# Murmeldyret/cubesat-APDS

Measured on AMD Instinct MI355X. Metric: frames/sec (detect+match+homography) 4k×4k tile vs 1M-desc DB; Mmatches/sec, higher is better.
Workload: dtype fp4 e2m1 operands / f32 accumulate = exact integer Hamming (match), f32 (AKAZE), f64 (homography solve)

## Files before the change

### cubesat-apds_amd/csrc/hamming_mfma.hip

```cpp
#include <atomic>
#include <memory>

#include "config.h"
#include "kernels.h"
#include "topk_keys.h"

namespace apds {

typedef int hm_v8i __attribute__((ext_vector_type(8)));
typedef float hm_f32x4 __attribute__((ext_vector_type(4)));
typedef uint32_t hm_u32x4 __attribute__((ext_vector_type(4)));

#ifndef APDS_HM_WAVES
#define APDS_HM_WAVES 8
#endif
static constexpr int HM_WAVES = APDS_HM_WAVES;
static constexpr int HM_TM = 16 * HM_WAVES;
#ifndef APDS_HM_WPE
#define APDS_HM_WPE 4
#endif
#ifndef APDS_HM_NC
#define APDS_HM_NC 3
#endif
static constexpr int HM_NC = APDS_HM_NC;
static constexpr int HM_Q = HM_WAVES * 16 * HM_NC;
static constexpr int HM_UNIT_SCALE = 0x7F7F7F7F;
static constexpr int HM_BIAS = 1024;

__device__ __forceinline__ uint32_t hm_spread8(uint32_t b, uint32_t nib) {
    uint32_t t = b & 0xFFu;
    t = (t | (t << 12)) & 0x000F000Fu;
    t = (t | (t << 6)) & 0x03030303u;
    t = (t | (t << 3)) & 0x11111111u;
    return t * nib;
}

__global__ __launch_bounds__(256) void hm_expand_rows_kernel(const uint32_t* __restrict__ rows, long long n, uint32_t nib, int bias, uint4* __restrict__ out,
                                                             float* __restrict__ pc) {
    APDS_RAISE_WAVE_PRIORITY();
    const long long i = (long long)blockIdx.x * 256 + threadIdx.x;
    const uint32_t d = i < n * 16 ? rows[i] : 0u;
    int v = __popc(d);
#pragma unroll
    for (int off = 8; off > 0; off >>= 1) v += __shfl_xor(v, off);
    if (i >= n * 16) return;
    out[i] = make_uint4(hm_spread8(d, nib), hm_spread8(d >> 8, nib), hm_spread8(d >> 16, nib), hm_spread8(d >> 24, nib));
    if ((threadIdx.x & 15) == 0) pc[i >> 4] = (float)(v + bias);
}

__global__ void hm_pad_rows_kernel(uint4* __restrict__ rows, float* __restrict__ pc, long long n, long long n_pad) {
    const long long i = n + (threadIdx.x >> 4);
    if (i >= n_pad) return;
    for (long long r = i; r < n_pad; r += 8) {
        rows[r * 16 + (threadIdx.x & 15)] = make_uint4(0, 0, 0, 0);
        if ((threadIdx.x & 15) == 0) pc[r] = INFINITY;
    }
}

__global__ void hm_thresholds_kernel(const uint64_t* __restrict__ topk, int K, const float* __restrict__ qpc, int nq, uint32_t* __restrict__ thr) {
    const int i = blockIdx.x * blockDim.x + threadIdx.x;
    if (i >= nq) return;
    const uint64_t k2 = topk[(size_t)i * K + K - 1];
    thr[i] = k2 == EMPTY_KEY ? 0x7F800000u : __float_as_uint((float)((int)key_rank(k2) - (int)qpc[i] + HM_BIAS));
}

struct HmTop2 {
    uint32_t d0, d1;
    uint32_t i0, i1;
};
__device__ __forceinline__ void hm_insert(HmTop2& b, uint32_t d, uint32_t idx) {
    if (d < b.d1) {
        if (d < b.d0) {
            b.d1 = b.d0;
            b.i1 = b.i0;
            b.d0 = d;
            b.i0 = idx;
        } else {
            b.d1 = d;
            b.i1 = idx;
        }
    }
}

__device__ __forceinline__ void hm_dma_rows(const unsigned char* tile_base, const int (&voff)[4], uint32_t lds_dst) {
    uint32_t keep;
    asm volatile(
        "s_mov_b32 %0, m0\n\t"
        "s_mov_b32 m0, %6\n\t"
        "s_nop 0\n\t"
        "global_load_lds_dwordx4 %1, %5\n\t"
        "global_load_lds_dwordx4 %2, %5 offset:1024\n\t"
        "global_load_lds_dwordx4 %3, %5 offset:2048\n\t"
        "global_load_lds_dwordx4 %4, %5 offset:3072\n\t"
        "s_mov_b32 m0, %0"
        : "=&s"(keep)
        : "v"(voff[0]), "v"(voff[1]), "v"(voff[2]), "v"(voff[3]), "s"(tile_base), "s"(lds_dst)
        : "memory");
}
__device__ __forceinline__ void hm_dma_popcounts(const float* src, int voff, uint32_t lds_dst) {
    uint32_t keep;
    asm volatile(
        "s_mov_b32 %0, m0\n\t"
        "s_mov_b32 m0, %3\n\t"
        "s_nop 0\n\t"
        "global_load_lds_dword %1, %2\n\t"
        "s_mov_b32 m0, %0"
        : "=&s"(keep)
        : "v"(voff), "s"(src), "s"(lds_dst)
        : "memory");
}
__device__ __forceinline__ void hm_dma_wait() { asm volatile("s_waitcnt vmcnt(0)" ::: "memory"); }
template <class T>
__device__ __forceinline__ void hm_settle(T& v) { asm volatile("" : "+v"(v)); }

template <int NC, int PRIO, class Rank>
__device__ __forceinline__ void hm_scan_tiles(const uint4* __restrict__ train_fp4, const float* __restrict__ tpc, int tile_begin, int tile_end,
// ... 45 lines not shown
            if (PRIO) __builtin_amdgcn_s_setprio(PRIO);
#pragma unroll
            for (int s = 0; s < 4; s++) {
                const hm_v8i A = {(int)a[s].x, (int)a[s].y, (int)a[s].z, (int)a[s].w, 0, 0, 0, 0};
#pragma unroll
                for (int c = 0; c < NC; c++) {
                    const hm_v8i Bv = {(int)B[c][s].x, (int)B[c][s].y, (int)B[c][s].z, (int)B[c][s].w, 0, 0, 0, 0};
                    acc[c] = __builtin_amdgcn_mfma_scale_f32_16x16x128_f8f6f4(A, Bv, s == 0 ? init : acc[c], 4, 4, 0, HM_UNIT_SCALE, 0, HM_UNIT_SCALE);
                }
            }
            if (PRIO) __builtin_amdgcn_s_setprio(0);
            if (rb + 1 < HM_TM / 16) {
                read_block(rb + 1);
            } else {
                hm_dma_wait();
                __syncthreads();
#pragma unroll
                for (int s = 0; s < 4; s++) ra[s] += buf ? -TILE_BYTES : TILE_BYTES;
                rn += buf ? -HM_TM * 4 : HM_TM * 4;
                read_block(0);
            }
#pragma unroll
            for (int c = 0; c < NC; c++) hm_settle(acc[c]);
            __builtin_amdgcn_sched_barrier(0);
            rank(acc, (uint32_t)(tile * HM_TM + rb * 16 + 4 * kq) + index_base);
        }
    }
}

struct HmItem {
    int split, q0, tile_begin, tile_end;
    int col, kq;
};
template <int NC>
__device__ __forceinline__ HmItem hm_work_item(int n_train, int tiles_per_split, int q_tiles, int splits) {
    const int tid = threadIdx.x, lane = tid & 63, wave = tid >> 6;
    HmItem w;
    int qtile;
    if ((splits & 7) == 0) {
        const int xcd = blockIdx.x & 7, j = blockIdx.x >> 3;
        w.split = xcd + 8 * (j / q_tiles);
        qtile = j % q_tiles;
    } else {
        w.split = blockIdx.x / q_tiles;
        qtile = blockIdx.x % q_tiles;
    }
    w.q0 = qtile * (HM_WAVES * 16 * NC) + wave * 16 * NC;
    const int n_tiles = (n_train + HM_TM - 1) / HM_TM;
    w.tile_begin = w.split * tiles_per_split, w.tile_end = min(n_tiles, w.tile_begin + tiles_per_split);
    w.col = lane & 15, w.kq = lane >> 4;
    return w;
}
template <int NC>
__device__ __forceinline__ void hm_load_queries(const uint4* query_fp4, const float* qpc, int nq, int q0, int col, int kq, uint4 (&B)[NC][4], float (&qq)[NC]) {
#pragma unroll
    for (int c = 0; c < NC; c++) {
        const int qi = min(q0 + 16 * c + col, nq - 1);
#pragma unroll
        for (int s = 0; s < 4; s++) B[c][s] = query_fp4[(size_t)qi * 16 + 4 * s + kq];
        qq[c] = qpc[qi];
    }
}
template <bool THR>
__device__ __forceinline__ uint32_t hm_start_value(const uint32_t* thr, int qi) {
    return THR ? thr[qi] : 0x7F800000u;
}
__device__ __forceinline__ uint32_t hm_distance(float qq, uint32_t d) { return (uint32_t)((int)(qq + __uint_as_float(d)) - HM_BIAS); }

template <int PRIO, bool THR>
__global__ __launch_bounds__(64 * HM_WAVES) __attribute__((amdgpu_waves_per_eu(APDS_HM_WPE, APDS_HM_WPE))) void hamming_mfma_kernel(const uint4* __restrict__ train_fp4, const float* __restrict__ tpc, int n_train,
                                                           const uint4* __restrict__ query_fp4, const float* __restrict__ qpc, int nq, int tiles_per_split,
                                                           int q_tiles, int splits, uint32_t index_base, const uint32_t* __restrict__ thr,
                                                           uint64_t* __restrict__ out) {
    const HmItem w = hm_work_item<HM_NC>(n_train, tiles_per_split, q_tiles, splits);
    const int split = w.split, q0 = w.q0, tile_begin = w.tile_begin, tile_end = w.tile_end, col = w.col, kq = w.kq;
    uint4 B[HM_NC][4];
    float qq[HM_NC];
    hm_load_queries<HM_NC>(query_fp4, qpc, nq, q0, col, kq, B, qq);
    HmTop2 best[HM_NC];
#pragma unroll
    for (int c = 0; c < HM_NC; c++) {
        best[c].d0 = hm_start_value<THR>(thr, min(q0 + 16 * c + col, nq - 1));
        hm_settle(best[c].d0), hm_settle(qq[c]);
        best[c].d1 = best[c].d0;
        best[c].i0 = best[c].i1 = 0xFFFFFFFFu;
    }

    if (tile_begin < tile_end) {
        hm_scan_tiles<HM_NC, PRIO>(train_fp4, tpc, tile_begin, tile_end, B, index_base, [&](const hm_f32x4 (&a)[HM_NC], uint32_t row0) {
            bool hit[HM_NC];
#pragma unroll
            for (int c = 0; c < HM_NC; c++) {
                const uint32_t mn = min(min(__float_as_uint(a[c][0]), __float_as_uint(a[c][1])), min(__float_as_uint(a[c][2]), __float_as_uint(a[c][3])));
                hit[c] = mn < best[c].d1;
            }
#pragma unroll
            for (int c = 0; c < HM_NC; c++)
                if (__any(hit[c])) {
#pragma unroll
                    for (int j = 0; j < 4; j++) hm_insert(best[c], __float_as_uint(a[c][j]), row0 + j);
                }
        });
    }
#pragma unroll
    for (int c = 0; c < HM_NC; c++) {
        HmTop2 b = best[c];
#pragma unroll
        for (int off = 16; off < 64; off <<= 1) {
            const uint32_t od0 = (uint32_t)__shfl_xor((int)b.d0, off), od1 = (uint32_t)__shfl_xor((int)b.d1, off);
            const uint32_t oi0 = (uint32_t)__shfl_xor((int)b.i0, off), oi1 = (uint32_t)__shfl_xor((int)b.i1, off);
            HmTop2 m = b;
            auto ins = [&](uint32_t d, uint32_t i) {
                if (i == 0xFFFFFFFFu) return;
                if (d < m.d0 || (d == m.d0 && i < m.i0)) {
                    m.d1 = m.d0;
                    m.i1 = m.i0;
                    m.d0 = d;
                    m.i0 = i;
                } else if ((d < m.d1 || (d == m.d1 && i < m.i1)) && i != m.i0) {
                    m.d1 = d;
                    m.i1 = i;
                }
            };
            ins(od0, oi0);
            ins(od1, oi1);
            b = m;
        }
        const int qi = q0 + 16 * c + col;
        if (kq == 0 && qi < nq) {
            uint64_t* o = out + ((size_t)split * nq + qi) * 2;
            o[0] = b.i0 == 0xFFFFFFFFu ? EMPTY_KEY : make_key(hm_distance(qq[c], b.d0), b.i0);
            o[1] = b.i1 == 0xFFFFFFFFu ? EMPTY_KEY : make_key(hm_distance(qq[c], b.d1), b.i1);
        }
    }
}

template <int K>
struct HmTopK {
    uint32_t d[K];
    uint32_t i[K];
};
template <int K>
__device__ __forceinline__ void hm_insert_k(HmTopK<K>& b, uint32_t d, uint32_t idx) {
#pragma unroll
    for (int j = K - 1; j > 0; j--) {
        const bool shift = d < b.d[j - 1], here = d < b.d[j];
        b.i[j] = shift ? b.i[j - 1] : (here ? idx : b.i[j]);
        b.d[j] = shift ? b.d[j - 1] : (here ? d : b.d[j]);
    }
    const bool first = d < b.d[0];
    b.i[0] = first ? idx : b.i[0];
    b.d[0] = first ? d : b.d[0];
}
__device__ __forceinline__ uint64_t hm_shfl_xor_u64(uint64_t v, int off) {
    return ((uint64_t)(uint32_t)__shfl_xor((int)(uint32_t)(v >> 32), off) << 32) | (uint32_t)__shfl_xor((int)(uint32_t)v, off);
}

#ifndef APDS_HM_NC_K4
#define APDS_HM_NC_K4 2
#endif
#ifndef APDS_HM_NC_K8
#define APDS_HM_NC_K8 2
#endif
template <int K>
struct HmShape {
    static constexpr int NC = K <= 4 ? APDS_HM_NC_K4 : APDS_HM_NC_K8;
    static constexpr int Q = HM_WAVES * 16 * NC;
};

template <int K, int NC, int PRIO, bool THR>
__global__ __launch_bounds__(64 * HM_WAVES) __attribute__((amdgpu_waves_per_eu(APDS_HM_WPE, APDS_HM_WPE))) void hamming_mfma_topk_kernel(
    const uint4* __restrict__ train_fp4, const float* __restrict__ tpc, int n_train, const uint4* __restrict__ query_fp4, const float* __restrict__ qpc, int nq,
    int tiles_per_split, int q_tiles, int splits, uint32_t index_base, const uint32_t* __restrict__ thr, uint64_t* __restrict__ out) {
    const HmItem w = hm_work_item<NC>(n_train, tiles_per_split, q_tiles, splits);
    const int split = w.split, q0 = w.q0, tile_begin = w.tile_begin, tile_end = w.tile_end, col = w.col, kq = w.kq;
    uint4 B[NC][4];
    float qq[NC];
    hm_load_queries<NC>(query_fp4, qpc, nq, q0, col, kq, B, qq);
    HmTopK<K> best[NC];
#pragma unroll
    for (int c = 0; c < NC; c++) {
        uint32_t start = hm_start_value<THR>(thr, min(q0 + 16 * c + col, nq - 1));
        hm_settle(start), hm_settle(qq[c]);
#pragma unroll
        for (int j = 0; j < K; j++) best[c].d[j] = start, best[c].i[j] = 0xFFFFFFFFu;
    }

    if (tile_begin < tile_end) {
        hm_scan_tiles<NC, PRIO>(train_fp4, tpc, tile_begin, tile_end, B, index_base, [&](const hm_f32x4 (&a)[NC], uint32_t row0) {
            bool hit[NC];
#pragma unroll
            for (int c = 0; c < NC; c++) {
                const uint32_t mn = min(min(__float_as_uint(a[c][0]), __float_as_uint(a[c][1])), min(__float_as_uint(a[c][2]), __float_as_uint(a[c][3])));
                hit[c] = mn < best[c].d[K - 1];
            }
#pragma unroll
            for (int c = 0; c < NC; c++)
                if (__any(hit[c])) {
#pragma unroll
                    for (int j = 0; j < 4; j++) {
                        const uint32_t v = __float_as_uint(a[c][j]);
                        if (__any(v < best[c].d[K - 1])) hm_insert_k<K>(best[c], v, row0 + j);
                    }
                }
        });
    }
#pragma unroll
    for (int c = 0; c < NC; c++) {
        uint64_t key[K];
#pragma unroll
        for (int j = 0; j < K; j++) key[j] = ((uint64_t)best[c].d[j] << 32) | best[c].i[j];
#pragma unroll
        for (int off = 16; off < 64; off <<= 1) {
            uint64_t other[K];
#pragma unroll
            for (int j = 0; j < K; j++) other[j] = hm_shfl_xor_u64(key[j], off);
#pragma unroll
            for (int j = 0; j < K; j++) key[j] = min(key[j], other[K - 1 - j]);
#pragma unroll
            for (int step = K / 2; step > 0; step >>= 1)
#pragma unroll
                for (int j = 0; j < K; j++)
                    if ((j & step) == 0) {
                        const uint64_t lo = min(key[j], key[j + step]), hi = max(key[j], key[j + step]);
                        key[j] = lo;
                        key[j + step] = hi;
                    }
        }
        const int qi = q0 + 16 * c + col;
        if (kq == 0 && qi < nq) {
            uint64_t* o = out + ((size_t)split * nq + qi) * K;
#pragma unroll
            for (int j = 0; j < K; j++) {
                const uint32_t d = key_rank(key[j]), i = key_index(key[j]);
                o[j] = i == 0xFFFFFFFFu ? EMPTY_KEY : make_key(hm_distance(qq[c], d), i);
            }
        }
    }
}

static int hm_list_len(int k) { return k <= 2 ? 2 : (k <= 4 ? 4 : 8); }
static int hm_queries_per_block(int K) { return K <= 2 ? HM_Q : (K <= 4 ? HmShape<4>::Q : HmShape<8>::Q); }

HmPlan hm_plan(int nq, long long nt, int K) {
    HmPlan p;
    p.q_tiles = ceil_div(nq, hm_queries_per_block(K));
    const int t_tiles = (int)ceil_div(nt, (long long)HM_TM);
    constexpr int SLOTS = 256 * (16 / HM_WAVES);
    constexpr int OVERHEAD = 4;
    const int max_splits = (int)std::max<long long>(1, std::min<long long>(std::min(t_tiles, 128), (32ll << 20) / std::max(K, 2) / std::max(nq, 1)));
    long long best_cost = -1;
    p.splits = 1;
    for (int sp = 1; sp <= max_splits; sp++) {
        const long long rounds = ceil_div((long long)p.q_tiles * sp, (long long)SLOTS);
        const long long cost = rounds * (ceil_div(t_tiles, sp) + OVERHEAD);
        if (best_cost < 0 || cost < best_cost) best_cost = cost, p.splits = sp;
    }
    if (config().match_mfma_xcd && t_tiles >= 64) {
        long long best8 = -1;
        int sp8 = 0;
        for (int sp = 8; sp <= std::min(max_splits, 32); sp += 8) {
            const long long rounds = ceil_div((long long)p.q_tiles * sp, (long long)SLOTS);
            const long long cost = rounds * (ceil_div(t_tiles, sp) + OVERHEAD);
            if (best8 < 0 || cost < best8) best8 = cost, sp8 = sp;
        }
        if (sp8 && best8 * 100 <= best_cost * 105) {
            p.splits = sp8;
            p.tiles_per_split = ceil_div(t_tiles, p.splits);
            return p;
        }
    }
    if (config().match_mfma_splits > 0) p.splits = std::min(t_tiles, config().match_mfma_splits);
    p.tiles_per_split = ceil_div(t_tiles, p.splits);
    p.splits = ceil_div(t_tiles, p.tiles_per_split);
    return p;
}

void hm_expand_device(const void* rows64, long long n, bool query, void* out_fp4, float* pc, hipStream_t s) {
    if (n <= 0) return;
    hipLaunchKernelGGL(hm_expand_rows_kernel, dim3((unsigned)ceil_div(n * 16, 256)), dim3(256), 0, s, static_cast<const uint32_t*>(rows64), n, query ? 0xCu : 0x2u,
                       query ? 0 : HM_BIAS, static_cast<uint4*>(out_fp4), pc);
    if (!query && hm_padded_rows(n) > n)
        hipLaunchKernelGGL(hm_pad_rows_kernel, dim3(1), dim3(128), 0, s, static_cast<uint4*>(out_fp4), pc, n, hm_padded_rows(n));
}
long long hm_padded_rows(long long n) { return ceil_div(n, (long long)HM_TM) * HM_TM; }
long long hm_sample_rows(long long nt) {
    const long long cap = config().match_mfma_sample;
    return (cap > 0 && nt >= 65536) ? std::min<long long>(cap, nt / 16 / HM_TM * HM_TM) / HM_TM * HM_TM : 0;
}

template <class... Kernel>
static void hm_opt_in_lds(std::atomic<bool> (&opted_dev)[64], Kernel... kernel) {
    std::atomic<bool>& opted = opted_dev[ctx().device & 63];
    if (opted.load()) return;
    (HIP_CHECK(hipFuncSetAttribute(reinterpret_cast<const void*>(kernel), hipFuncAttributeMaxDynamicSharedMemorySize, 160 * 1024)), ...);
    opted.store(true);
}

template <int K, class Go>
static void hm_scan_k_launch(Go&& go, bool thr) {
    constexpr int NC = HmShape<K>::NC;
    static std::atomic<bool> opted_dev[64];
    hm_opt_in_lds(opted_dev, &hamming_mfma_topk_kernel<K, NC, 0, false>, &hamming_mfma_topk_kernel<K, NC, 2, false>,
                  &hamming_mfma_topk_kernel<K, NC, 0, true>, &hamming_mfma_topk_kernel<K, NC, 2, true>);
    const bool prio = config().match_mfma_prio > 0;
    if (thr) prio ? go(&hamming_mfma_topk_kernel<K, NC, 2, true>) : go(&hamming_mfma_topk_kernel<K, NC, 0, true>);
    else prio ? go(&hamming_mfma_topk_kernel<K, NC, 2, false>) : go(&hamming_mfma_topk_kernel<K, NC, 0, false>);
}

void hm_scan_device(const void* q_fp4, const float* qpc, int nq, const void* t_fp4, const float* tpc, long long nt, const HmPlan& p, uint32_t index_base,
                    uint64_t* parts, hipStream_t s, const uint32_t* thr, bool timed, int K) {
    APDS_REQUIRE(K <= 2 || K == 4 || K == 8, APDS_ERR_ASSERT, "the matrix-core matcher keeps lists of 2, 4 or 8");
    const size_t lds = (size_t)2 * HM_TM * 256 + 2 * HM_TM * sizeof(float) + (size_t)std::max(0, config().match_mfma_lds_pad);
    auto go = [&](auto kernel) {
        hipLaunchKernelGGL(kernel, dim3((unsigned)p.q_tiles * p.splits), dim3(64 * HM_WAVES), lds, s, static_cast<const uint4*>(t_fp4), tpc, (int)nt,
                           static_cast<const uint4*>(q_fp4), qpc, nq, p.tiles_per_split, p.q_tiles, p.splits, index_base, thr, parts);
    };
    std::unique_ptr<KernelTimer> timer, timer_k;
    if (timed) timer.reset(new KernelTimer("hamming_topk", s));
    if (timed && K > 2) timer_k.reset(new KernelTimer("hamming_topk_mfma_k", s));
    if (K == 4) return hm_scan_k_launch<4>(go, thr != nullptr);
    if (K == 8) return hm_scan_k_launch<8>(go, thr != nullptr);
    static std::atomic<bool> opted_dev[64];
    hm_opt_in_lds(opted_dev, &hamming_mfma_kernel<0, false>, &hamming_mfma_kernel<1, false>, &hamming_mfma_kernel<2, false>, &hamming_mfma_kernel<3, false>,
                  &hamming_mfma_kernel<0, true>, &hamming_mfma_kernel<1, true>, &hamming_mfma_kernel<2, true>, &hamming_mfma_kernel<3, true>);
    const int prio = std::max(0, std::min(3, config().match_mfma_prio));
    if (thr) {
        switch (prio) {
            case 0: go(&hamming_mfma_kernel<0, true>); break;
            case 1: go(&hamming_mfma_kernel<1, true>); break;
            case 2: go(&hamming_mfma_kernel<2, true>); break;
            default: go(&hamming_mfma_kernel<3, true>); break;
        }
    } else {
        switch (prio) {
            case 0: go(&hamming_mfma_kernel<0, false>); break;
            case 1: go(&hamming_mfma_kernel<1, false>); break;
            case 2: go(&hamming_mfma_kernel<2, false>); break;
            default: go(&hamming_mfma_kernel<3, false>); break;
        }
    }
}

void* hm_train_create(const void* rows64, long long n, hipStream_t s) {
    APDS_REQUIRE(rows64 && n > 0 && n < (1ll << 31), APDS_ERR_ASSERT, "an expanded train set needs rows");
    HmTrain* t = new HmTrain();
    t->device = ctx().device;
    t->src = rows64;
    t->n = n;
    if (hipMalloc(&t->rows, (size_t)hm_padded_rows(n) * 256) != hipSuccess || hipMalloc(reinterpret_cast<void**>(&t->pc), (size_t)hm_padded_rows(n) * 4) != hipSuccess) {
        (void)hipGetLastError();
        if (t->rows) (void)hipFree(t->rows);
        delete t;
        fail(APDS_ERR_NOMEM, "no device memory for the expanded train rows");
    }
    hm_expand_device(rows64, n, false, t->rows, t->pc, s);
    HIP_CHECK(hipStreamSynchronize(s));
    return t;
}
void hm_train_destroy(void* h) {
    HmTrain* t = static_cast<HmTrain*>(h);
    if (!t) return;
    int previous = -1;
    if (hipGetDevice(&previous) != hipSuccess) previous = -1;
    (void)hipSetDevice(t->device);
    (void)hipDeviceSynchronize();
    if (t->rows) (void)hipFree(t->rows);
    if (t->pc) (void)hipFree(t->pc);
    delete t;
    if (previous >= 0) (void)hipSetDevice(previous);
}

static void hm_topk_expanded(const void* q, int nq, const void* t4, const float* tp, long long nt, uint32_t index_base, int k, uint64_t* out, hipStream_t s) {
    ThreadCtx& c = ctx();
    void* q4 = c.alloc((size_t)nq * 256);
    float* qp = c.alloc_n<float>(nq);
    {
        KernelTimer timer("hamming_topk_sample", s);
        hm_expand_device(q, nq, true, q4, qp, s);
    }
    const long long sample = hm_sample_rows(nt);
    const int K = hm_list_len(k);
    uint64_t* topk = k == K ? out : c.alloc_n<uint64_t>((size_t)nq * K);
    const HmPlan p = hm_plan(nq, nt - sample, K);
    const int lists = p.splits + (sample ? 1 : 0);
    uint64_t* parts = lists == 1 ? topk : c.alloc_n<uint64_t>((size_t)lists * nq * K);
    uint32_t* thr = nullptr;
    if (sample) {
        const HmPlan pa = hm_plan(nq, sample, K);
        uint64_t* parts_a = c.alloc_n<uint64_t>((size_t)pa.splits * nq * K);
        uint64_t* topk_a = parts + (size_t)p.splits * nq * K;
        thr = c.alloc_n<uint32_t>(nq);
        KernelTimer timer("hamming_topk_sample", s);
        hm_scan_device(q4, qp, nq, t4, tp, sample, pa, index_base, parts_a, s, nullptr, false, K);
        if (pa.splits > 1) merge_topk_device(parts_a, pa.splits, nq, K, topk_a, s);
        else HIP_CHECK(hipMemcpyAsync(topk_a, parts_a, (size_t)nq * K * 8, hipMemcpyDeviceToDevice, s));
        hipLaunchKernelGGL(hm_thresholds_kernel, dim3(ceil_div(nq, 256)), dim3(256), 0, s, (const uint64_t*)topk_a, K, (const float*)qp, nq, thr);
    }
    hm_scan_device(q4, qp, nq, static_cast<const char*>(t4) + (size_t)sample * 256, tp + sample, nt - sample, p, index_base + (uint32_t)sample, parts, s, thr,
                   true, K);
    if (lists > 1) merge_topk_device(parts, lists, nq, K, topk, s);
    if (k != K) take_first_columns_device(topk, nq, K, k, out, s);
    HIP_CHECK(hipGetLastError());
}

void hamming_mfma_topk_device(const void* q, int nq, const void* t, long long nt, uint32_t index_base, int k, uint64_t* out, hipStream_t s) {
    APDS_REQUIRE(k >= 1 && k <= 8, APDS_ERR_ASSERT, "the matrix-core matcher serves 1 <= k <= 8");
    APDS_REQUIRE(nq > 0 && nt > 0 && nt < (1ll << 31), APDS_ERR_ASSERT, "the matrix-core matcher needs queries and train rows");
    ThreadCtx& c = ctx();
    void* t4 = c.alloc((size_t)hm_padded_rows(nt) * 256);
    float* tp = c.alloc_n<float>(hm_padded_rows(nt));
    {
        KernelTimer timer("hamming_topk_sample", s);
        hm_expand_device(t, nt, false, t4, tp, s);
    }
    hm_topk_expanded(q, nq, t4, tp, nt, index_base, k, out, s);
}

void hamming_mfma_topk_train_device(const void* q, int nq, const void* train, uint32_t index_base, int k, uint64_t* out, hipStream_t s) {
    const HmTrain* t = static_cast<const HmTrain*>(train);
    APDS_REQUIRE(t && k >= 1 && k <= 8 && nq > 0, APDS_ERR_ASSERT, "the matrix-core matcher needs an expanded train set, queries and 1 <= k <= 8");
    hm_topk_expanded(q, nq, t->rows, t->pc, t->n, index_base, k, out, s);
}

}
```

### cubesat-apds_amd/csrc/kernels.h

```cpp
#pragma once
#include <atomic>
#include "common.h"

namespace apds {

void hamming_topk_device(const void* q, int nq, const void* t, long long nt, uint32_t index_base, int k, uint64_t* out, hipStream_t s, int backend = 0);
void* topk_split_create();
void topk_split_destroy(void* state);
void topk_split_prepass(void* state, const void* q, int nq, const void* t, long long nt, uint32_t index_base, int k, hipStream_t s);
void topk_split_scan(void* state, const void* q, const void* t, hipStream_t s);
void topk_split_merge(void* state, uint32_t index_base, uint64_t* out, hipStream_t s);
void topk_split_use_train(void* state, const void* hm_train);
void pack_rows_device(const void* src, long long n, int desc_bytes, long long src_stride, void* dst, hipStream_t s);
std::atomic<int>& match_lds_cap();
std::atomic<int>& last_scan_launch_lds();
void set_thread_scan_cap(int bytes);

void merge_topk_device(const uint64_t* parts, int nparts, int nq, int k, uint64_t* out, hipStream_t s);
void take_first_columns_device(const uint64_t* in, int nq, int kin, int kout, uint64_t* out, hipStream_t s);

void hamming_mfma_topk_device(const void* q, int nq, const void* t, long long nt, uint32_t index_base, int k, uint64_t* out, hipStream_t s);
struct HmPlan {
    int q_tiles, splits, tiles_per_split;
};
struct HmTrain {
    int device = 0;
    const void* src = nullptr;
    long long n = 0;
    void* rows = nullptr;
    float* pc = nullptr;
};
HmPlan hm_plan(int nq, long long nt, int K = 2);
long long hm_padded_rows(long long n);
void hm_expand_device(const void* rows64, long long n, bool query, void* out_fp4, float* pc, hipStream_t s);
void hm_scan_device(const void* q_fp4, const float* qpc, int nq, const void* t_fp4, const float* tpc, long long nt, const HmPlan& p, uint32_t index_base,
                    uint64_t* parts, hipStream_t s, const uint32_t* thr = nullptr, bool timed = true, int K = 2);
long long hm_sample_rows(long long nt);
void* hm_train_create(const void* rows64, long long n, hipStream_t s);
void hm_train_destroy(void* train);
void hamming_mfma_topk_train_device(const void* q, int nq, const void* train, uint32_t index_base, int k, uint64_t* out, hipStream_t s);

int* scan_flags_device(const uint8_t* flags, int n, int** total_dev, hipStream_t s);
int ratio_filter_device(const uint64_t* keys, int nq, int k, float fs, apds_dmatch* out, hipStream_t s);
int cross_check_device(const uint64_t* train_best, long long n_train, int nq, apds_dmatch* out, hipStream_t s);

double valu_popcount_peak_device();
int valu_peak_modes();
const char* valu_peak_mode_name(int mode);
void valu_peak_device(int mode, int waves_per_simd, double* lane_ops_per_s, double* cycles_per_inst);

int akaze_extract_device(const void* img, int rows, int cols, int channels, size_t stride, int max_points, apds_keypoint* kps,
                         uint8_t* desc64, int capacity, hipStream_t s);
int akaze_extract_batch_device(const void* img, int n_img, size_t img_bstride, int rows, int cols, int channels, size_t stride, int max_points,
                               apds_keypoint* kps, uint8_t* desc64, int capacity, int* counts, hipStream_t s);

void points_from_matches_device(const apds_keypoint* kp1, int n1, const apds_keypoint* kp2, int n2, const apds_dmatch* m, int nm,
                                int bug_compatible, float* pts1, float* pts2, int* err_flag, hipStream_t s);
void rgba_to_bgra_device(const uint8_t* rgba, size_t n_pixels, uint8_t* bgra, hipStream_t s);
int count_nonzero_device(const uint8_t* bytes, int n, int* count_dev, hipStream_t s);

void band_merger_device(const float* r, const float* g, const float* b, size_t n, const double* mm, int bgra, uint8_t* out, hipStream_t s);
void warp_perspective_device(const uint8_t* src, int rows, int cols, const double* M, int dst_rows, int dst_cols, uint8_t* dst, hipStream_t s);
void warp_perspective_any_device(const void* src, int rows, int cols, int channels, int elem_bytes, const double* M, int dst_rows, int dst_cols, void* dst,
                                 hipStream_t s);
int world_coordinates_device(const double* xy, int n, const double* dgt_host, const double* egt_host, const double* elev, int ew, int eh, double* xyz,
                             hipStream_t s);

struct Mosaic;
void mosaic_check_window(const Mosaic* m, int level, const int32_t* xy0, int n_tiles, int win_w, int win_h, int out_w, int out_h, int resample);
void mosaic_read_device(const Mosaic* m, const int32_t* xy0, int n_tiles, int win_w, int win_h, int out_w, int out_h, int resample, float* out, hipStream_t s);
void mosaic_min_max(Mosaic* m, double* minmax6);

int find_homography_device(const float* src, const float* dst, int n, int method, double thr, int max_iters, double confidence,
                           double* H_host, uint8_t* mask_dev, hipStream_t s);

void l2_row_norms_device(const float* x, long long n, int dim, float* out, hipStream_t s);
void l2_topk_device(const float* q, int nq, const float* t, long long nt, int dim, uint32_t index_base, int k, uint64_t* out, hipStream_t s);
bool l2_topk_screen_device(const float* q, int nq, const float* t, long long nt, int dim, uint32_t index_base, int k, uint64_t* out, hipStream_t s,
                           double* candidates_per_query);

int find_homography_rho_device(const float* src, const float* dst, int n, double thr, int max_iters, double confidence, double* H_host, uint8_t* mask_dev,
                               hipStream_t s);

int pnp_ransac_device(const double* obj_xyz, const double* img_xy, int n, const double* K, int iterations, float reproj_thr, double confidence, int method,
                      double* rvec, double* tvec, int32_t* inliers, int* n_inliers, hipStream_t s);
int pnp_ransac_core(const float* obj_dev, const float* img_dev, int n, const double* K, int iterations, float reproj_thr, double confidence, int method,
                    double* rvec, double* tvec, int32_t* inliers, int* n_inliers, hipStream_t s);
int pnp_checked_method(int n, int method);
// ... 9 lines not shown
```

### cubesat-apds_amd/csrc/match_hamming.hip

```cpp
#include <atomic>

#include "config.h"
#include "kernels.h"
#include "popcount_row.h"
#include "topk_keys.h"

namespace apds {

typedef uint32_t u32x4 __attribute__((ext_vector_type(4)));

static constexpr int INF_THR = 1 << 20;
static constexpr uint32_t NO_INDEX = 0xFFFFFFFFu;
static constexpr int PART_ROW_BITS = 22;
template <int T, int K>
struct PartRecord {
    static constexpr int SLOTS = T * K;
    static constexpr int HEADER = 2 * SLOTS;
    static constexpr int PITCH = HEADER + 64 * SLOTS;
};

#ifndef APDS_PAIR_NOP
#define APDS_PAIR_NOP 1
#endif
template <int T>
// ... 433 lines not shown
                   reinterpret_cast<uint32_t*>(buf + L.off_parts), L.p, s, "hamming_topk", floor_keys, floor_base);
}

template <int K>
static void scan_merge(const ScanLayout& L, const char* buf, uint32_t index_base, uint64_t* out, hipStream_t s) {
    merge_records_launch<K>(reinterpret_cast<const uint32_t*>(buf + L.off_parts), L.p, index_base + (uint32_t)L.sample,
                            L.sample ? reinterpret_cast<const uint64_t*>(buf + L.off_sample_keys) : nullptr, L.nq, out, s);
    HIP_CHECK(hipGetLastError());
}

template <int K>
static void topk_device_k(const void* q, int nq, const void* t, long long nt, uint32_t index_base, uint64_t* out, hipStream_t s) {
    const ScanLayout L = scan_layout<K>(nq, nt, false);
    char* buf = static_cast<char*>(ctx().alloc(L.bytes));
    scan_prepass<K>(L, buf, q, t, index_base, s);
    scan_main<K>(L, buf, q, t, s);
    scan_merge<K>(L, buf, index_base, out, s);
}

__global__ void gather_pages_kernel(const uint64_t* __restrict__ pages, int nq, int n_pages, int k, uint64_t* __restrict__ out) {
    const long long i = (long long)blockIdx.x * blockDim.x + threadIdx.x;
    if (i >= (long long)nq * k) return;
    const int q = (int)(i / k), c = (int)(i - (long long)q * k);
    const int page = c >> 4;
    out[i] = page < n_pages ? pages[((size_t)page * nq + q) * 16 + (c & 15)] : EMPTY_KEY;
}

static void topk_paged_device(const void* q, int nq, const void* t, long long nt, uint32_t index_base, int k, uint64_t* out, hipStream_t s) {
    constexpr int K = 16;
    ThreadCtx& c = ctx();
    const int n_pages = (int)std::min<long long>(ceil_div(k, K), ceil_div(nt, K));
    const ScanLayout L = scan_layout<K>(nq, nt, true);
    char* buf = static_cast<char*>(c.alloc(L.bytes));
    uint64_t* pages = c.alloc_n<uint64_t>((size_t)n_pages * nq * K);
    for (int j = 0; j < n_pages; j++) {
        const uint64_t* floor_keys = j ? pages + (size_t)(j - 1) * nq * K : nullptr;
        scan_prepass<K>(L, buf, q, t, index_base, s, floor_keys, index_base);
        scan_main<K>(L, buf, q, t, s, floor_keys, index_base + (uint32_t)L.sample);
        scan_merge<K>(L, buf, index_base, pages + (size_t)j * nq * K, s);
    }
    hipLaunchKernelGGL(gather_pages_kernel, dim3((unsigned)ceil_div((long long)nq * k, 256)), dim3(256), 0, s, (const uint64_t*)pages, nq, n_pages, k, out);
    HIP_CHECK(hipGetLastError());
}

struct TopkSplitState {
    int device = 0;
    char* buf = nullptr;
    size_t cap = 0;
    ScanLayout L{};
    bool mfma = false;
    HmPlan hp{};
    const HmTrain* shared_train = nullptr;
    uint32_t index_base_mfma = 0;
    size_t off_q4 = 0, off_qp = 0, off_t4 = 0, off_tp = 0, off_lists = 0, off_top2 = 0;
    const void* t4 = nullptr;
    const float* tp = nullptr;
};

static void split_reserve(TopkSplitState& st, size_t need) {
    if (need <= st.cap) return;
    HIP_CHECK(hipDeviceSynchronize());
    if (st.buf) (void)hipFree(st.buf);
    st.buf = nullptr;
    st.cap = 0;
    const size_t want = need + need / 4;
    HIP_CHECK(hipMalloc(reinterpret_cast<void**>(&st.buf), want));
    st.cap = want;
}

static void split_prepass_mfma(TopkSplitState& st, const void* q, int nq, const void* t, long long nt, int k, hipStream_t s) {
    st.mfma = true;
    st.L = ScanLayout{};
    st.L.nq = nq, st.L.k = k, st.L.nt = nt;
    st.hp = hm_plan(nq, nt);
    const bool shared = st.shared_train && st.shared_train->src == t && st.shared_train->n == nt;
    size_t need = 0;
    auto take = [&](size_t bytes) {
        const size_t o = need;
        need += (bytes + 255) & ~(size_t)255;
        return o;
    };
    st.off_q4 = take((size_t)nq * 256);
    st.off_qp = take((size_t)nq * 4);
    st.off_lists = take((size_t)st.hp.splits * nq * 16);
    st.off_top2 = take((size_t)nq * 16);
    if (!shared) {
        st.off_t4 = take((size_t)hm_padded_rows(nt) * 256);
        st.off_tp = take((size_t)hm_padded_rows(nt) * 4);
    }
    split_reserve(st, need);
    KernelTimer timer("hamming_topk_sample", s);
    hm_expand_device(q, nq, true, st.buf + st.off_q4, reinterpret_cast<float*>(st.buf + st.off_qp), s);
    if (shared) {
        st.t4 = st.shared_train->rows;
        st.tp = st.shared_train->pc;
    } else {
        hm_expand_device(t, nt, false, st.buf + st.off_t4, reinterpret_cast<float*>(st.buf + st.off_tp), s);
        st.t4 = st.buf + st.off_t4;
        st.tp = reinterpret_cast<const float*>(st.buf + st.off_tp);
    }
    HIP_CHECK(hipGetLastError());
}
static void split_scan_mfma(TopkSplitState& st, hipStream_t s) {
    hm_scan_device(st.buf + st.off_q4, reinterpret_cast<const float*>(st.buf + st.off_qp), st.L.nq, st.t4, st.tp, st.L.nt, st.hp, st.index_base_mfma,
                   reinterpret_cast<uint64_t*>(st.buf + st.off_lists), s);
}
static void split_merge_mfma(TopkSplitState& st, uint64_t* out, hipStream_t s) {
    const int nq = st.L.nq, k = st.L.k;
    const uint64_t* parts = reinterpret_cast<const uint64_t*>(st.buf + st.off_lists);
    uint64_t* top2 = k == 2 ? out : reinterpret_cast<uint64_t*>(st.buf + st.off_top2);
    if (st.hp.splits > 1) merge_topk_device(parts, st.hp.splits, nq, 2, top2, s);
    else if (k == 2) HIP_CHECK(hipMemcpyAsync(out, parts, (size_t)nq * 16, hipMemcpyDeviceToDevice, s));
    else top2 = const_cast<uint64_t*>(parts);
    if (k == 1) take_first_columns_device(top2, nq, 2, 1, out, s);
    HIP_CHECK(hipGetLastError());
}

template <int K>
static void split_prepass_k(TopkSplitState& st, const void* q, int nq, const void* t, long long nt, uint32_t index_base, hipStream_t s) {
    st.L = scan_layout<K>(nq, nt, false);
    split_reserve(st, st.L.bytes);
    scan_prepass<K>(st.L, st.buf, q, t, index_base, s);
}

void* topk_split_create() {
    TopkSplitState* st = new TopkSplitState();
    st->device = ctx().device;
    return st;
}
void topk_split_destroy(void* h) {
    TopkSplitState* st = static_cast<TopkSplitState*>(h);
    if (!st) return;
    int previous = -1;
    if (hipGetDevice(&previous) != hipSuccess) previous = -1;
    (void)hipSetDevice(st->device);
    (void)hipDeviceSynchronize();
    if (st->buf) (void)hipFree(st->buf);
    delete st;
    if (previous >= 0) (void)hipSetDevice(previous);
}
void topk_split_prepass(void* h, const void* q, int nq, const void* t, long long nt, uint32_t index_base, int k, hipStream_t s) {
    APDS_REQUIRE(h, APDS_ERR_BAD_ARG, "null scan state");
    APDS_REQUIRE(k == 1 || k == 2, APDS_ERR_ASSERT, "the split scan serves k = 1 and k = 2 (what the crate surface consumes, lib.rs:107-111)");
    APDS_REQUIRE(nq > 0 && nt > 0 && nt < (1ll << 31), APDS_ERR_ASSERT, "the split scan needs queries and train rows");
    TopkSplitState& st = *static_cast<TopkSplitState*>(h);
    if (config().match_mfma) {
        st.index_base_mfma = index_base;
        split_prepass_mfma(st, q, nq, t, nt, k, s);
        return;
    }
    st.mfma = false;
    if (k == 1) split_prepass_k<1>(st, q, nq, t, nt, index_base, s);
    else split_prepass_k<2>(st, q, nq, t, nt, index_base, s);
}
void topk_split_use_train(void* h, const void* hm_train) {
    APDS_REQUIRE(h, APDS_ERR_BAD_ARG, "null scan state");
    static_cast<TopkSplitState*>(h)->shared_train = static_cast<const HmTrain*>(hm_train);
}
void topk_split_scan(void* h, const void* q, const void* t, hipStream_t s) {
    APDS_REQUIRE(h, APDS_ERR_BAD_ARG, "null scan state");
    TopkSplitState& st = *static_cast<TopkSplitState*>(h);
    APDS_REQUIRE(st.L.nq > 0, APDS_ERR_ASSERT, "scan before pre-pass");
    if (st.mfma) {
        split_scan_mfma(st, s);
        return;
    }
    if (st.L.k == 1) scan_main<1>(st.L, st.buf, q, t, s);
    else scan_main<2>(st.L, st.buf, q, t, s);
}
void topk_split_merge(void* h, uint32_t index_base, uint64_t* out, hipStream_t s) {
    APDS_REQUIRE(h && out, APDS_ERR_BAD_ARG, "null scan state / output");
    TopkSplitState& st = *static_cast<TopkSplitState*>(h);
    APDS_REQUIRE(st.L.nq > 0, APDS_ERR_ASSERT, "merge before pre-pass");
    if (st.mfma) {
        APDS_REQUIRE(index_base == st.index_base_mfma, APDS_ERR_ASSERT, "the merge's index base differs from the pre-pass's");
        split_merge_mfma(st, out, s);
        return;
    }
    if (st.L.k == 1) scan_merge<1>(st.L, st.buf, index_base, out, s);
    else scan_merge<2>(st.L, st.buf, index_base, out, s);
}

void hamming_topk_device(const void* q, int nq, const void* t, long long nt, uint32_t index_base, int k, uint64_t* out,
                         hipStream_t s, int backend) {
    APDS_REQUIRE(k >= 1, APDS_ERR_ASSERT, "top-k needs k >= 1");
    APDS_REQUIRE(nt < (1ll << 31), APDS_ERR_ASSERT, "train set too large for one call; shard it");
    APDS_REQUIRE(!(backend == 3 && k > 8), APDS_ERR_ASSERT, "backend 3 (matrix cores) serves k <= 8");
    if (nq <= 0) return;
    if (nt <= 0) {
        HIP_CHECK(hipMemsetAsync(out, 0xFF, (size_t)nq * k * 8, s));
        return;
    }
    if (k > 16) {
        topk_paged_device(q, nq, t, nt, index_base, k, out, s);
        return;
    }
    APDS_REQUIRE(backend >= 0 && backend <= 3 && !(backend == 2 && k > 2) && !(backend == 3 && k > 8), APDS_ERR_ASSERT,
                 "backend: 0 default, 1 vector ALU, 2 matrix cores (k <= 2), 3 matrix cores (k <= 8)");
    if (backend == 2 || backend == 3 || (backend == 0 && config().match_mfma && k <= std::max(2, config().match_mfma_kmax))) {
        hamming_mfma_topk_device(q, nq, t, nt, index_base, k, out, s);
        return;
    }
    const int K = k <= 2 ? k : (k <= 4 ? 4 : (k <= 8 ? 8 : 16));
    uint64_t* dst = K == k ? out : ctx().alloc_n<uint64_t>((size_t)nq * K);
    switch (K) {
        case 1: topk_device_k<1>(q, nq, t, nt, index_base, dst, s); break;
        case 2: topk_device_k<2>(q, nq, t, nt, index_base, dst, s); break;
        case 4: topk_device_k<4>(q, nq, t, nt, index_base, dst, s); break;
        case 8: topk_device_k<8>(q, nq, t, nt, index_base, dst, s); break;
        default: topk_device_k<16>(q, nq, t, nt, index_base, dst, s); break;
    }
    if (K != k) {
        take_first_columns_device(dst, nq, K, k, out, s);
        HIP_CHECK(hipGetLastError());
    }
}

// ... 10 lines not shown
```

### cubesat-apds_amd/csrc/topk_merge.hip

```cpp
#include "kernels.h"
#include "topk_keys.h"

namespace apds {

template <int K>
__global__ void merge_topk_kernel(const uint64_t* __restrict__ parts_keys, int parts, int nq, uint64_t* __restrict__ out) {
    APDS_RAISE_WAVE_PRIORITY();
    const int qi = blockIdx.x * blockDim.x + threadIdx.x;
    if (qi >= nq) return;
    uint64_t best[K];
#pragma unroll
    for (int k = 0; k < K; k++) best[k] = EMPTY_KEY;
    constexpr int U = K <= 2 ? 8 : 2;
    int p = 0;
    for (; p + U <= parts; p += U) {
        uint64_t v[U][K];
#pragma unroll
        for (int u = 0; u < U; u++)
#pragma unroll
            for (int k = 0; k < K; k++) v[u][k] = parts_keys[((size_t)(p + u) * nq + qi) * K + k];
#pragma unroll
        for (int u = 0; u < U; u++)
#pragma unroll
            for (int k = 0; k < K; k++) topk_insert<K>(best, v[u][k]);
    }
    for (; p < parts; p++)
#pragma unroll
        for (int k = 0; k < K; k++) topk_insert<K>(best, parts_keys[((size_t)p * nq + qi) * K + k]);
#pragma unroll
    for (int k = 0; k < K; k++) out[(size_t)qi * K + k] = best[k];
}

__global__ void merge_topk_any_kernel(const uint64_t* __restrict__ parts_keys, int parts, int nq, int k, uint64_t* __restrict__ out) {
    APDS_RAISE_WAVE_PRIORITY();
    const int qi = blockIdx.x * blockDim.x + threadIdx.x;
    if (qi >= nq) return;
    uint16_t cur[64];
    for (int p = 0; p < parts; p++) cur[p] = 0;
    for (int j = 0; j < k; j++) {
        uint64_t best = EMPTY_KEY;
        int arg = -1;
        for (int p = 0; p < parts; p++) {
            if (cur[p] >= k) continue;
            const uint64_t v = parts_keys[((size_t)p * nq + qi) * k + cur[p]];
            if (v < best) best = v, arg = p;
        }
        out[(size_t)qi * k + j] = best;
        if (arg >= 0) cur[arg]++;
    }
}

__global__ void take_first_columns_kernel(const uint64_t* __restrict__ in, int nq, int kin, int kout, uint64_t* __restrict__ out) {
    const long long i = (long long)blockIdx.x * blockDim.x + threadIdx.x;
    if (i >= (long long)nq * kout) return;
    const int q = (int)(i / kout), c = (int)(i - (long long)q * kout);
    out[i] = in[(size_t)q * kin + c];
}

template <int K>
static void merge_launch(const uint64_t* parts, int nparts, int nq, uint64_t* out, hipStream_t s) {
    hipLaunchKernelGGL((merge_topk_kernel<K>), dim3(ceil_div(nq, 256)), dim3(256), 0, s, parts, nparts, nq, out);
}

void merge_topk_device(const uint64_t* parts, int nparts, int nq, int k, uint64_t* out, hipStream_t s) {
    if (nq <= 0) return;
    switch (k) {
        case 1: merge_launch<1>(parts, nparts, nq, out, s); break;
        case 2: merge_launch<2>(parts, nparts, nq, out, s); break;
        case 4: merge_launch<4>(parts, nparts, nq, out, s); break;
        case 8: merge_launch<8>(parts, nparts, nq, out, s); break;
        case 16: merge_launch<16>(parts, nparts, nq, out, s); break;
        default:
            APDS_REQUIRE(k >= 1 && k <= 4096 && nparts <= 64, APDS_ERR_ASSERT, "merge supports 1 <= k <= 4096 over at most 64 lists");
            hipLaunchKernelGGL(merge_topk_any_kernel, dim3(ceil_div(nq, 64)), dim3(64), 0, s, parts, nparts, nq, k, out);
    }
    HIP_CHECK(hipGetLastError());
}

void take_first_columns_device(const uint64_t* in, int nq, int kin, int kout, uint64_t* out, hipStream_t s) {
    if (nq <= 0) return;
    hipLaunchKernelGGL(take_first_columns_kernel, dim3(ceil_div((long long)nq * kout, 256)), dim3(256), 0, s, in, nq, kin, kout, out);
}

}
```

Before: 154.4.

## Expand query descriptors inside the scan kernels and fuse threshold computation into merge

Query rows are no longer pre-expanded to fp4 with a separate kernel and buffer. Each scan kernel now reads the raw 64-byte descriptors, spreads them into fp4 operands in registers, and computes the popcount with lane shuffles. The sample-pass merge and threshold computation are fused into one kernel that recomputes the query popcount, which also removes the memcpy when there is a single split. This cuts launches and global traffic, at the cost of repeating the expansion work in every scan block.

```diff
diff --git a/cubesat-apds_amd/csrc/hamming_mfma.hip b/cubesat-apds_amd/csrc/hamming_mfma.hip
--- a/cubesat-apds_amd/csrc/hamming_mfma.hip
+++ b/cubesat-apds_amd/csrc/hamming_mfma.hip
@@ -55,13 +55,6 @@
         rows[r * 16 + (threadIdx.x & 15)] = make_uint4(0, 0, 0, 0);
         if ((threadIdx.x & 15) == 0) pc[r] = INFINITY;
     }
-}
-
-__global__ void hm_thresholds_kernel(const uint64_t* __restrict__ topk, int K, const float* __restrict__ qpc, int nq, uint32_t* __restrict__ thr) {
-    const int i = blockIdx.x * blockDim.x + threadIdx.x;
-    if (i >= nq) return;
-    const uint64_t k2 = topk[(size_t)i * K + K - 1];
-    thr[i] = k2 == EMPTY_KEY ? 0x7F800000u : __float_as_uint((float)((int)key_rank(k2) - (int)qpc[i] + HM_BIAS));
 }
 
 struct HmTop2 {
@@ -213,13 +206,20 @@
     return w;
 }
 template <int NC>
-__device__ __forceinline__ void hm_load_queries(const uint4* query_fp4, const float* qpc, int nq, int q0, int col, int kq, uint4 (&B)[NC][4], float (&qq)[NC]) {
+__device__ __forceinline__ void hm_load_queries(const uint32_t* __restrict__ query64, int nq, int q0, int col, int kq, uint4 (&B)[NC][4], float (&qq)[NC]) {
 #pragma unroll
     for (int c = 0; c < NC; c++) {
         const int qi = min(q0 + 16 * c + col, nq - 1);
-#pragma unroll
-        for (int s = 0; s < 4; s++) B[c][s] = query_fp4[(size_t)qi * 16 + 4 * s + kq];
-        qq[c] = qpc[qi];
+        int pc = 0;
+#pragma unroll
+        for (int s = 0; s < 4; s++) {
+            const uint32_t d = query64[(size_t)qi * 16 + 4 * s + kq];
+            B[c][s] = make_uint4(hm_spread8(d, 0xCu), hm_spread8(d >> 8, 0xCu), hm_spread8(d >> 16, 0xCu), hm_spread8(d >> 24, 0xCu));
+            pc += __popc(d);
+        }
+        pc += __shfl_xor(pc, 16);
+        pc += __shfl_xor(pc, 32);
+        qq[c] = (float)pc;
     }
 }
 template <bool THR>
@@ -230,14 +230,14 @@
 
 template <int PRIO, bool THR>
 __global__ __launch_bounds__(64 * HM_WAVES) __attribute__((amdgpu_waves_per_eu(APDS_HM_WPE, APDS_HM_WPE))) void hamming_mfma_kernel(const uint4* __restrict__ train_fp4, const float* __restrict__ tpc, int n_train,
-                                                           const uint4* __restrict__ query_fp4, const float* __restrict__ qpc, int nq, int tiles_per_split,
+                                                           const uint32_t* __restrict__ query64, int nq, int tiles_per_split,
                                                            int q_tiles, int splits, uint32_t index_base, const uint32_t* __restrict__ thr,
                                                            uint64_t* __restrict__ out) {
     const HmItem w = hm_work_item<HM_NC>(n_train, tiles_per_split, q_tiles, splits);
     const int split = w.split, q0 = w.q0, tile_begin = w.tile_begin, tile_end = w.tile_end, col = w.col, kq = w.kq;
     uint4 B[HM_NC][4];
     float qq[HM_NC];
-    hm_load_queries<HM_NC>(query_fp4, qpc, nq, q0, col, kq, B, qq);
+    hm_load_queries<HM_NC>(query64, nq, q0, col, kq, B, qq);
     HmTop2 best[HM_NC];
 #pragma unroll
     for (int c = 0; c < HM_NC; c++) {
@@ -331,13 +331,13 @@
 
 template <int K, int NC, int PRIO, bool THR>
 __global__ __launch_bounds__(64 * HM_WAVES) __attribute__((amdgpu_waves_per_eu(APDS_HM_WPE, APDS_HM_WPE))) void hamming_mfma_topk_kernel(
-    const uint4* __restrict__ train_fp4, const float* __restrict__ tpc, int n_train, const uint4* __restrict__ query_fp4, const float* __restrict__ qpc, int nq,
+    const uint4* __restrict__ train_fp4, const float* __restrict__ tpc, int n_train, const uint32_t* __restrict__ query64, int nq,
     int tiles_per_split, int q_tiles, int splits, uint32_t index_base, const uint32_t* __restrict__ thr, uint64_t* __restrict__ out) {
     const HmItem w = hm_work_item<NC>(n_train, tiles_per_split, q_tiles, splits);
     const int split = w.split, q0 = w.q0, tile_begin = w.tile_begin, tile_end = w.tile_end, col = w.col, kq = w.kq;
     uint4 B[NC][4];
     float qq[NC];
-    hm_load_queries<NC>(query_fp4, qpc, nq, q0, col, kq, B, qq);
+    hm_load_queries<NC>(query64, nq, q0, col, kq, B, qq);
     HmTopK<K> best[NC];
 #pragma unroll
     for (int c = 0; c < NC; c++) {
@@ -437,11 +437,11 @@
     return p;
 }
 
-void hm_expand_device(const void* rows64, long long n, bool query, void* out_fp4, float* pc, hipStream_t s) {
+void hm_expand_device(const void* rows64, long long n, void* out_fp4, float* pc, hipStream_t s) {
     if (n <= 0) return;
-    hipLaunchKernelGGL(hm_expand_rows_kernel, dim3((unsigned)ceil_div(n * 16, 256)), dim3(256), 0, s, static_cast<const uint32_t*>(rows64), n, query ? 0xCu : 0x2u,
-                       query ? 0 : HM_BIAS, static_cast<uint4*>(out_fp4), pc);
-    if (!query && hm_padded_rows(n) > n)
+    hipLaunchKernelGGL(hm_expand_rows_kernel, dim3((unsigned)ceil_div(n * 16, 256)), dim3(256), 0, s, static_cast<const uint32_t*>(rows64), n, 0x2u, HM_BIAS,
+                       static_cast<uint4*>(out_fp4), pc);
+    if (hm_padded_rows(n) > n)
         hipLaunchKernelGGL(hm_pad_rows_kernel, dim3(1), dim3(128), 0, s, static_cast<uint4*>(out_fp4), pc, n, hm_padded_rows(n));
 }
 long long hm_padded_rows(long long n) { return ceil_div(n, (long long)HM_TM) * HM_TM; }
@@ -469,13 +469,13 @@
     else prio ? go(&hamming_mfma_topk_kernel<K, NC, 2, false>) : go(&hamming_mfma_topk_kernel<K, NC, 0, false>);
 }
 
-void hm_scan_device(const void* q_fp4, const float* qpc, int nq, const void* t_fp4, const float* tpc, long long nt, const HmPlan& p, uint32_t index_base,
+void hm_scan_device(const void* q64, int nq, const void* t_fp4, const float* tpc, long long nt, const HmPlan& p, uint32_t index_base,
                     uint64_t* parts, hipStream_t s, const uint32_t* thr, bool timed, int K) {
     APDS_REQUIRE(K <= 2 || K == 4 || K == 8, APDS_ERR_ASSERT, "the matrix-core matcher keeps lists of 2, 4 or 8");
     const size_t lds = (size_t)2 * HM_TM * 256 + 2 * HM_TM * sizeof(float) + (size_t)std::max(0, config().match_mfma_lds_pad);
     auto go = [&](auto kernel) {
         hipLaunchKernelGGL(kernel, dim3((unsigned)p.q_tiles * p.splits), dim3(64 * HM_WAVES), lds, s, static_cast<const uint4*>(t_fp4), tpc, (int)nt,
-                           static_cast<const uint4*>(q_fp4), qpc, nq, p.tiles_per_split, p.q_tiles, p.splits, index_base, thr, parts);
+                           static_cast<const uint32_t*>(q64), nq, p.tiles_per_split, p.q_tiles, p.splits, index_base, thr, parts);
     };
     std::unique_ptr<KernelTimer> timer, timer_k;
     if (timed) timer.reset(new KernelTimer("hamming_topk", s));
@@ -515,7 +515,7 @@
         delete t;
         fail(APDS_ERR_NOMEM, "no device memory for the expanded train rows");
     }
-    hm_expand_device(rows64, n, false, t->rows, t->pc, s);
+    hm_expand_device(rows64, n, t->rows, t->pc, s);
     HIP_CHECK(hipStreamSynchronize(s));
     return t;
 }
@@ -534,12 +534,6 @@
 
 static void hm_topk_expanded(const void* q, int nq, const void* t4, const float* tp, long long nt, uint32_t index_base, int k, uint64_t* out, hipStream_t s) {
     ThreadCtx& c = ctx();
-    void* q4 = c.alloc((size_t)nq * 256);
-    float* qp = c.alloc_n<float>(nq);
-    {
-        KernelTimer timer("hamming_topk_sample", s);
-        hm_expand_device(q, nq, true, q4, qp, s);
-    }
     const long long sample = hm_sample_rows(nt);
     const int K = hm_list_len(k);
     uint64_t* topk = k == K ? out : c.alloc_n<uint64_t>((size_t)nq * K);
@@ -553,12 +547,10 @@
         uint64_t* topk_a = parts + (size_t)p.splits * nq * K;
         thr = c.alloc_n<uint32_t>(nq);
         KernelTimer timer("hamming_topk_sample", s);
-        hm_scan_device(q4, qp, nq, t4, tp, sample, pa, index_base, parts_a, s, nullptr, false, K);
-        if (pa.splits > 1) merge_topk_device(parts_a, pa.splits, nq, K, topk_a, s);
-        else HIP_CHECK(hipMemcpyAsync(topk_a, parts_a, (size_t)nq * K * 8, hipMemcpyDeviceToDevice, s));
-        hipLaunchKernelGGL(hm_thresholds_kernel, dim3(ceil_div(nq, 256)), dim3(256), 0, s, (const uint64_t*)topk_a, K, (const float*)qp, nq, thr);
-    }
-    hm_scan_device(q4, qp, nq, static_cast<const char*>(t4) + (size_t)sample * 256, tp + sample, nt - sample, p, index_base + (uint32_t)sample, parts, s, thr,
+        hm_scan_device(q, nq, t4, tp, sample, pa, index_base, parts_a, s, nullptr, false, K);
+        merge_topk_thresholds_device(parts_a, pa.splits, nq, K, q, HM_BIAS, topk_a, thr, s);
+    }
+    hm_scan_device(q, nq, static_cast<const char*>(t4) + (size_t)sample * 256, tp + sample, nt - sample, p, index_base + (uint32_t)sample, parts, s, thr,
                    true, K);
     if (lists > 1) merge_topk_device(parts, lists, nq, K, topk, s);
     if (k != K) take_first_columns_device(topk, nq, K, k, out, s);
@@ -573,7 +565,7 @@
     float* tp = c.alloc_n<float>(hm_padded_rows(nt));
     {
         KernelTimer timer("hamming_topk_sample", s);
-        hm_expand_device(t, nt, false, t4, tp, s);
+        hm_expand_device(t, nt, t4, tp, s);
     }
     hm_topk_expanded(q, nq, t4, tp, nt, index_base, k, out, s);
 }
diff --git a/cubesat-apds_amd/csrc/kernels.h b/cubesat-apds_amd/csrc/kernels.h
--- a/cubesat-apds_amd/csrc/kernels.h
+++ b/cubesat-apds_amd/csrc/kernels.h
@@ -18,6 +18,7 @@
 
 void merge_topk_device(const uint64_t* parts, int nparts, int nq, int k, uint64_t* out, hipStream_t s);
 void take_first_columns_device(const uint64_t* in, int nq, int kin, int kout, uint64_t* out, hipStream_t s);
+void merge_topk_thresholds_device(const uint64_t* parts, int nparts, int nq, int k, const void* query64, int bias, uint64_t* out, uint32_t* thr, hipStream_t s);
 
 void hamming_mfma_topk_device(const void* q, int nq, const void* t, long long nt, uint32_t index_base, int k, uint64_t* out, hipStream_t s);
 struct HmPlan {
@@ -32,8 +33,8 @@
 };
 HmPlan hm_plan(int nq, long long nt, int K = 2);
 long long hm_padded_rows(long long n);
-void hm_expand_device(const void* rows64, long long n, bool query, void* out_fp4, float* pc, hipStream_t s);
-void hm_scan_device(const void* q_fp4, const float* qpc, int nq, const void* t_fp4, const float* tpc, long long nt, const HmPlan& p, uint32_t index_base,
+void hm_expand_device(const void* rows64, long long n, void* out_fp4, float* pc, hipStream_t s);
+void hm_scan_device(const void* q64, int nq, const void* t_fp4, const float* tpc, long long nt, const HmPlan& p, uint32_t index_base,
                     uint64_t* parts, hipStream_t s, const uint32_t* thr = nullptr, bool timed = true, int K = 2);
 long long hm_sample_rows(long long nt);
 void* hm_train_create(const void* rows64, long long n, hipStream_t s);
diff --git a/cubesat-apds_amd/csrc/match_hamming.hip b/cubesat-apds_amd/csrc/match_hamming.hip
--- a/cubesat-apds_amd/csrc/match_hamming.hip
+++ b/cubesat-apds_amd/csrc/match_hamming.hip
@@ -509,7 +509,7 @@
     HmPlan hp{};
     const HmTrain* shared_train = nullptr;
     uint32_t index_base_mfma = 0;
-    size_t off_q4 = 0, off_qp = 0, off_t4 = 0, off_tp = 0, off_lists = 0, off_top2 = 0;
+    size_t off_t4 = 0, off_tp = 0, off_lists = 0, off_top2 = 0;
     const void* t4 = nullptr;
     const float* tp = nullptr;
 };
@@ -537,8 +537,6 @@
         need += (bytes + 255) & ~(size_t)255;
         return o;
     };
-    st.off_q4 = take((size_t)nq * 256);
-    st.off_qp = take((size_t)nq * 4);
     st.off_lists = take((size_t)st.hp.splits * nq * 16);
     st.off_top2 = take((size_t)nq * 16);
     if (!shared) {
@@ -546,20 +544,19 @@
         st.off_tp = take((size_t)hm_padded_rows(nt) * 4);
     }
     split_reserve(st, need);
-    KernelTimer timer("hamming_topk_sample", s);
-    hm_expand_device(q, nq, true, st.buf + st.off_q4, reinterpret_cast<float*>(st.buf + st.off_qp), s);
     if (shared) {
         st.t4 = st.shared_train->rows;
         st.tp = st.shared_train->pc;
     } else {
-        hm_expand_device(t, nt, false, st.buf + st.off_t4, reinterpret_cast<float*>(st.buf + st.off_tp), s);
+        KernelTimer timer("hamming_topk_sample", s);
+        hm_expand_device(t, nt, st.buf + st.off_t4, reinterpret_cast<float*>(st.buf + st.off_tp), s);
         st.t4 = st.buf + st.off_t4;
         st.tp = reinterpret_cast<const float*>(st.buf + st.off_tp);
     }
     HIP_CHECK(hipGetLastError());
 }
-static void split_scan_mfma(TopkSplitState& st, hipStream_t s) {
-    hm_scan_device(st.buf + st.off_q4, reinterpret_cast<const float*>(st.buf + st.off_qp), st.L.nq, st.t4, st.tp, st.L.nt, st.hp, st.index_base_mfma,
+static void split_scan_mfma(TopkSplitState& st, const void* q, hipStream_t s) {
+    hm_scan_device(q, st.L.nq, st.t4, st.tp, st.L.nt, st.hp, st.index_base_mfma,
                    reinterpret_cast<uint64_t*>(st.buf + st.off_lists), s);
 }
 static void split_merge_mfma(TopkSplitState& st, uint64_t* out, hipStream_t s) {
@@ -619,7 +616,7 @@
     TopkSplitState& st = *static_cast<TopkSplitState*>(h);
     APDS_REQUIRE(st.L.nq > 0, APDS_ERR_ASSERT, "scan before pre-pass");
     if (st.mfma) {
-        split_scan_mfma(st, s);
+        split_scan_mfma(st, q, s);
         return;
     }
     if (st.L.k == 1) scan_main<1>(st.L, st.buf, q, t, s);
diff --git a/cubesat-apds_amd/csrc/topk_merge.hip b/cubesat-apds_amd/csrc/topk_merge.hip
--- a/cubesat-apds_amd/csrc/topk_merge.hip
+++ b/cubesat-apds_amd/csrc/topk_merge.hip
@@ -4,11 +4,7 @@
 namespace apds {
 
 template <int K>
-__global__ void merge_topk_kernel(const uint64_t* __restrict__ parts_keys, int parts, int nq, uint64_t* __restrict__ out) {
-    APDS_RAISE_WAVE_PRIORITY();
-    const int qi = blockIdx.x * blockDim.x + threadIdx.x;
-    if (qi >= nq) return;
-    uint64_t best[K];
+__device__ __forceinline__ void merge_lists(const uint64_t* __restrict__ parts_keys, int parts, int nq, int qi, uint64_t (&best)[K]) {
 #pragma unroll
     for (int k = 0; k < K; k++) best[k] = EMPTY_KEY;
     constexpr int U = K <= 2 ? 8 : 2;
@@ -27,8 +23,36 @@
     for (; p < parts; p++)
 #pragma unroll
         for (int k = 0; k < K; k++) topk_insert<K>(best, parts_keys[((size_t)p * nq + qi) * K + k]);
+}
+
+template <int K>
+__global__ void merge_topk_kernel(const uint64_t* __restrict__ parts_keys, int parts, int nq, uint64_t* __restrict__ out) {
+    APDS_RAISE_WAVE_PRIORITY();
+    const int qi = blockIdx.x * blockDim.x + threadIdx.x;
+    if (qi >= nq) return;
+    uint64_t best[K];
+    merge_lists<K>(parts_keys, parts, nq, qi, best);
 #pragma unroll
     for (int k = 0; k < K; k++) out[(size_t)qi * K + k] = best[k];
+}
+
+template <int K>
+__global__ __launch_bounds__(256) void merge_topk_thresholds_kernel(const uint64_t* __restrict__ parts_keys, int parts, int nq, const uint4* __restrict__ query64, int bias,
+                                             uint64_t* __restrict__ out, uint32_t* __restrict__ thr) {
+    APDS_RAISE_WAVE_PRIORITY();
+    const int qi = blockIdx.x * blockDim.x + threadIdx.x;
+    if (qi >= nq) return;
+    uint4 row[4];
+#pragma unroll
+    for (int j = 0; j < 4; j++) row[j] = query64[(size_t)qi * 4 + j];
+    uint64_t best[K];
+    merge_lists<K>(parts_keys, parts, nq, qi, best);
+#pragma unroll
+    for (int k = 0; k < K; k++) out[(size_t)qi * K + k] = best[k];
+    int pc = 0;
+#pragma unroll
+    for (int j = 0; j < 4; j++) pc += __popc(row[j].x) + __popc(row[j].y) + __popc(row[j].z) + __popc(row[j].w);
+    thr[qi] = best[K - 1] == EMPTY_KEY ? 0x7F800000u : __float_as_uint((float)((int)key_rank(best[K - 1]) - pc + bias));
 }
 
 __global__ void merge_topk_any_kernel(const uint64_t* __restrict__ parts_keys, int parts, int nq, int k, uint64_t* __restrict__ out) {
@@ -77,6 +101,20 @@
     HIP_CHECK(hipGetLastError());
 }
 
+void merge_topk_thresholds_device(const uint64_t* parts, int nparts, int nq, int k, const void* query64, int bias, uint64_t* out, uint32_t* thr, hipStream_t s) {
+    if (nq <= 0) return;
+    auto go = [&](auto kernel) {
+        hipLaunchKernelGGL(kernel, dim3(ceil_div(nq, 256)), dim3(256), 0, s, parts, nparts, nq, static_cast<const uint4*>(query64), bias, out, thr);
+    };
+    switch (k) {
+        case 2: go(&merge_topk_thresholds_kernel<2>); break;
+        case 4: go(&merge_topk_thresholds_kernel<4>); break;
+        case 8: go(&merge_topk_thresholds_kernel<8>); break;
+        default: APDS_REQUIRE(false, APDS_ERR_ASSERT, "the matrix-core matcher keeps lists of 2, 4 or 8");
+    }
+    HIP_CHECK(hipGetLastError());
+}
+
 void take_first_columns_device(const uint64_t* in, int nq, int kin, int kout, uint64_t* out, hipStream_t s) {
     if (nq <= 0) return;
     hipLaunchKernelGGL(take_first_columns_kernel, dim3(ceil_div((long long)nq * kout, 256)), dim3(256), 0, s, in, nq, kin, kout, out);
```

After: 154.2. About the same (-0.1%).
